# xmed-lab/GL-Fusion

Hardware: AMD Instinct MI355X
Metric: clips/sec fwd+bwd (B=4, 3 views x16x112x112) per GPU, weak scaling (higher is better)
Workload: dtype f32 (amax-scaled split-fp16 x3 MFMA, fp32 accumulate: fp32-equivalent); 1 GPU; C2: (B,V,T,H,W)=(4,3,16,112,112) per GPU, views 1/3/4, fp32 train() fwd + sum-BCE + bwd; global_batch_clips=4, frames_per_view_per_gpu=64, precision=f16x3, parallelism=single GPU, ranks_in_collective=1

## Files before the change

gl-fusion_amd/csrc/conv_api.hip:

```cpp
#include "gemm_common.h"
#include <cstring>

namespace {

int conv_out(int h, int k, int stride, int pad, int dil) { return (h + 2 * pad - dil * (k - 1) - 1) / stride + 1; }

unsigned tap_mask_of(int gather, int hd, int wd, int hs, int ws, int kh, int kw, int stride, int pad, int dil) {
    auto axis = [&](int nd, int ns, int k, bool* ok) {
        for (int t = 0; t < k; ++t) {
            ok[t] = false;
            for (int y = 0; y < nd && !ok[t]; ++y) {
                if (gather == 1) {
                    const int sy = y * stride - pad + t * dil;
                    ok[t] = sy >= 0 && sy < ns;
                } else {
                    const int v = y + pad - t * dil;
                    ok[t] = v >= 0 && v % stride == 0 && v / stride < ns;
                }
            }
        }
    };
    bool vy[32], vx[32];
    axis(hd, hs, kh, vy);
    axis(wd, ws, kw, vx);
// ... 30 lines not shown
        long long best = want;
        double best_score = -1.0;
        long long lo = want / 2 > 1 ? want / 2 : 1, up = want * 2;
        if (up > cap) up = cap;
        if (up > hi) up = hi;
        if (up < 1) up = 1;
        for (long long s = lo; s <= up; ++s) {
            const long long b = wg * s;
            const double score = (double)b / ((double)((b + 255) / 256) * 256.0) - 0.004 * (double)s;
            if (score > best_score) { best = s; best_score = score; }
        }
        want = best;
    }
    if (want > cap) want = cap;
    if (want > hi) want = hi;
    return (int)(want < 1 ? 1 : want);
}

int check_params(const glf_conv_params* p, const char* who) {
    GLF_REQUIRE(p != nullptr, GLF_ERR_NULL, "%s: null parameter block", who);
    GLF_REQUIRE(p->n > 0 && p->h > 0 && p->w > 0 && p->cin > 0 && p->cout > 0, GLF_ERR_BAD_SHAPE, "%s: extents must be > 0", who);
    GLF_REQUIRE(p->kh >= 1 && p->kw >= 1 && p->kh * p->kw <= 32 && p->stride >= 1 && p->dil >= 1 && p->pad >= 0, GLF_ERR_BAD_SHAPE,
                "%s: bad kernel geometry (kh*kw must be <= 32)", who);
    GLF_REQUIRE(p->precision >= 0 && p->precision <= 4, GLF_ERR_UNSUPPORTED, "%s: precision must be 0..4", who);
    GLF_REQUIRE(conv_out(p->h, p->kh, p->stride, p->pad, p->dil) > 0 && conv_out(p->w, p->kw, p->stride, p->pad, p->dil) > 0, GLF_ERR_BAD_SHAPE,
                "%s: empty output", who);
    return GLF_OK;
}

int effective_precision(const glf_conv_params* p) { return p->precision >= 1 ? p->precision - 1 : glf::precision(); }

constexpr double THR_FWD = 0.8, THR_DGRAD = 0.8, THR_DGRAD_F16 = 0.35, THR_WGRAD = 0.8, THR_REGION = 0.8;

void fill_geo(glf_gemm_params& g, const glf_conv_params* p, bool to_input, int ho, int wo) {
    g.n_img = p->n;
    g.kh = p->kh; g.kw = p->kw; g.stride = p->stride; g.pad = p->pad; g.dil = p->dil;
    if (to_input) { g.hs = ho; g.ws = wo; g.hd = p->h; g.wd = p->w; }
    else { g.hs = p->h; g.ws = p->w; g.hd = ho; g.wd = wo; }
}

}

extern "C" int glf_conv2d_plan(const glf_conv_params* p, int pass, glf_conv_plan* plan) {
    if (int rc = check_params(p, "conv2d_plan")) return rc;
    GLF_REQUIRE(plan != nullptr && pass >= 0 && pass <= 2, GLF_ERR_NULL, "conv2d_plan: plan missing or pass not in {0 fwd, 1 dgrad, 2 wgrad}");
    std::memset(plan, 0, sizeof(*plan));
    const int prec = effective_precision(p);
    const int ho = conv_out(p->h, p->kh, p->stride, p->pad, p->dil), wo = conv_out(p->w, p->kw, p->stride, p->pad, p->dil);
    const int taps = p->kh * p->kw;
    const bool plain = taps == 1 && p->stride == 1 && p->pad == 0;
    plan->ho = ho; plan->wo = wo; plan->taps = taps; plan->plain = plain; plan->split = 1;
    if (pass == 0 || pass == 2) {
        const unsigned mask = plain ? 1u : tap_mask_of(1, ho, wo, p->h, p->w, p->kh, p->kw, p->stride, p->pad, p->dil);
        const int kept = __builtin_popcount(mask);
        const double frac = (plain || p->stride != 1) ? 1.0 : rect_fraction(1, ho, wo, p->h, p->w, p->kw, p->pad, p->dil, mask);
        plan->tap_mask = mask; plan->kept_taps = kept;
        if (pass == 0) {
            plan->M = p->n * ho * wo; plan->N = p->cout; plan->K = p->cin;
            plan->rect = (!plain && taps > 1 && p->stride == 1 && kept > 1 && frac < THR_FWD) ? 1 : 0;
            plan->zero_fill = plan->rect == 1;
            plan->colstats_ok = prec >= 2 && p->cin % 32 == 0 && p->cout % 4 == 0 && plan->rect == 0;
        } else {
            const bool rect = !plain && taps > 1 && p->stride == 1 && kept > 1 && frac < THR_WGRAD;
            const long long rows_o = (long long)p->n * ho * wo;
            long long eff = rect ? (long long)((double)rows_o * frac) : rows_o;
            if (eff < 512) eff = 512;
            plan->M = p->cout; plan->N = p->cin; plan->K = (int)rows_o;
            plan->rect = rect ? 1 : 0;
            plan->split = tn_split(eff, p->cout, p->cin, kept, prec);
            if (rect) {
                long long s2 = (long long)((double)plan->split / (2.0 * (frac > 0.02 ? frac : 0.02)) + 0.999);
                if (s2 < plan->split) s2 = plan->split;
                const long long cap = rows_o / 512 > 1 ? rows_o / 512 : 1;
                if (s2 > cap) s2 = cap;
                if (s2 > 65535) s2 = 65535;
                plan->split = (int)(s2 < 1 ? 1 : s2);
            }
            plan->workspace_bytes = plan->split > 1 ? (int64_t)plan->split * kept * p->cout * p->cin * (int64_t)sizeof(float) : 0;
            plan->zero_fill = mask != ((taps == 32) ? 0xffffffffu : ((1u << taps) - 1u));
        }
    } else {
        const unsigned mask = plain ? 1u : tap_mask_of(2, p->h, p->w, ho, wo, p->kh, p->kw, p->stride, p->pad, p->dil);
        const int kept = __builtin_popcount(mask);
        const double frac = (plain || p->stride != 1) ? 1.0 : rect_fraction(2, p->h, p->w, ho, wo, p->kw, p->pad, p->dil, mask);
        plan->tap_mask = mask; plan->kept_taps = kept;
        plan->M = p->n * p->h * p->w; plan->N = p->cin; plan->K = p->cout;
        const bool region = prec >= 2 && !plain && kept > 1 && taps == 9 && p->kh == 3 && p->stride == 1 && p->pad == p->dil && ho == p->h &&
                            wo == p->w && p->cout % 32 == 0 && frac < THR_REGION;
        const double thr = prec >= 2 ? THR_DGRAD_F16 : THR_DGRAD;
        plan->rect = region ? 2 : ((!plain && taps > 1 && p->stride == 1 && kept > 1 && frac < thr) ? 1 : 0);
        plan->zero_fill = plan->rect == 1 || mask == 0;
    }
    return GLF_OK;
}

extern "C" int glf_conv2d_fwd(const float* x, const float* w_tap, const float* bias, float* y, const glf_conv_params* p, glf_stream_t s) {
    glf_conv_plan pl;
    if (int rc = glf_conv2d_plan(p, 0, &pl)) return rc;
    GLF_REQUIRE(x && w_tap && y, GLF_ERR_NULL, "conv2d_fwd: null argument");
    GLF_REQUIRE(!(pl.rect && bias), GLF_ERR_UNSUPPORTED, "conv2d_fwd: a bias on a conv that runs as per-tap rectangles is not built (none on the path)");
    GLF_REQUIRE(!p->colstats || pl.colstats_ok, GLF_ERR_UNSUPPORTED, "conv2d_fwd: colstats cannot be honoured for this conv / precision (see glf_conv_plan.colstats_ok)");
    if (pl.zero_fill) {
        hipError_t e = hipMemsetAsync(y, 0, (size_t)pl.M * pl.N * sizeof(float), glf::S(s));
        if (e != hipSuccess) return glf::fail(GLF_ERR_LAUNCH, "conv2d_fwd: hipMemsetAsync: %s", hipGetErrorString(e));
    }
    glf_gemm_params g;
    std::memset(&g, 0, sizeof(g));
    g.M = pl.M; g.N = pl.N; g.K = pl.K; g.lda = p->cin; g.ldb = p->cin; g.ldc = p->cout;
    g.taps = pl.taps; g.tap_mask = pl.tap_mask; g.tap_stride_b = (int64_t)p->cout * p->cin;
    g.gather = pl.plain ? 0 : 1;
    fill_geo(g, p, false, pl.ho, pl.wo);
    if (pl.plain) { g.n_img = 1; g.hs = g.ws = g.hd = g.wd = 1; g.kh = g.kw = 1; g.stride = 1; g.pad = 0; g.dil = 1; }
    g.batch = 1; g.alpha = 1.f; g.split = 1; g.rect = pl.rect;
    g.amax_a = p->amax_x; g.amax_b = p->amax_w; g.amax_c = p->amax_out; g.colstats = p->colstats; g.precision = p->precision;
    if (pl.rect == 1 && effective_precision(p) == 0) {
        for (unsigned mm = pl.tap_mask; mm; mm &= mm - 1) {
            g.tap_mask = mm & (~mm + 1u);
            if (int rc = glf_gemm_nt(x, w_tap, bias, y, &g, s)) return rc;
        }
        return GLF_OK;
    }
    return glf_gemm_nt(x, w_tap, bias, y, &g, s);
}

extern "C" int glf_conv2d_dgrad(const float* dy, const float* w_tap, const float* w_tap_t, float* dx, const glf_conv_params* p, glf_stream_t s) {
    glf_conv_plan pl;
    if (int rc = glf_conv2d_plan(p, 1, &pl)) return rc;
    GLF_REQUIRE(dy && dx && (w_tap || w_tap_t), GLF_ERR_NULL, "conv2d_dgrad: null argument");
    if (pl.zero_fill) {
        hipError_t e = hipMemsetAsync(dx, 0, (size_t)pl.M * pl.N * sizeof(float), glf::S(s));
        if (e != hipSuccess) return glf::fail(GLF_ERR_LAUNCH, "conv2d_dgrad: hipMemsetAsync: %s", hipGetErrorString(e));
        if (pl.tap_mask == 0) return GLF_OK;
    }
    const int prec = effective_precision(p);
    glf_gemm_params g;
    std::memset(&g, 0, sizeof(g));
    g.M = pl.M; g.N = pl.N; g.K = pl.K; g.lda = p->cout; g.ldc = p->cin;
    g.taps = pl.taps; g.tap_mask = pl.tap_mask; g.tap_stride_b = (int64_t)p->cout * p->cin;
    g.gather = pl.plain ? 0 : 2;
    fill_geo(g, p, true, pl.ho, pl.wo);
    if (pl.plain) { g.n_img = 1; g.hs = g.ws = g.hd = g.wd = 1; g.kh = g.kw = 1; g.stride = 1; g.pad = 0; g.dil = 1; }
    g.batch = 1; g.alpha = 1.f; g.split = 1; g.rect = pl.rect;
    g.amax_a = p->amax_dy; g.amax_b = p->amax_w; g.amax_c = p->amax_out; g.precision = p->precision;
    if (prec >= 1 && p->cout % 32 == 0 && w_tap_t) {
        g.ldb = p->cout;
        return glf_gemm_nt(dy, w_tap_t, nullptr, dx, &g, s);
// ... 35 lines not shown
```

gl-fusion_amd/csrc/gemm_common.h:

```cpp
#pragma once
#include "glf_common.h"

namespace glf {
struct Geo { int n_img, hs, ws, hd, wd, kh, kw, stride, pad, dil; };

struct GemmArgs {
    const float* A; const float* B; const float* bias; float* C;
    int M, N, K, lda, ldb, ldc, taps;
    unsigned tap_mask;
    long long tap_stride_b;
    int gather;
    Geo g;
    long long bsa, bsb, bsc;
    float alpha;
    int accumulate, split;
    int tiles_m, tiles_n;
    int vec_a, vec_b;
    int rect;
    const float* amax_a; const float* amax_b;
    const float* zeros;
    float* amax_c;
    double* colstats;
    float* colmax;
    float* partial;
// ... 69 lines not shown
}

__host__ __device__ inline void tap_rect(int gather, int tap, int kw, int pad, int dil, int hs, int ws, int hd, int wd,
                                         int& y0, int& y1, int& x0, int& x1) {
    const int ky = tap / kw, kx = tap - ky * kw;
    const int oy = (gather == 1) ? pad - ky * dil : ky * dil - pad;
    const int ox = (gather == 1) ? pad - kx * dil : kx * dil - pad;
    y0 = oy > 0 ? oy : 0;           y1 = hs + oy < hd ? hs + oy : hd;
    x0 = ox > 0 ? ox : 0;           x1 = ws + ox < wd ? ws + ox : wd;
    if (y1 < y0) y1 = y0;
    if (x1 < x0) x1 = x0;
}

__host__ __device__ inline void axis_band(int gather, int b, int d, int h, int& lo, int& hi, unsigned& taps) {
    int e1 = d < h - d ? d : h - d, e2 = d < h - d ? h - d : d;
    e1 = e1 < 0 ? 0 : (e1 > h ? h : e1);
    e2 = e2 < 0 ? 0 : (e2 > h ? h : e2);
    lo = b == 0 ? 0 : (b == 1 ? e1 : e2);
    hi = b == 0 ? e1 : (b == 1 ? e2 : h);
    const unsigned first = gather == 1 ? 0b110u : 0b011u, last = gather == 1 ? 0b011u : 0b110u;
    taps = b == 0 ? first : (b == 2 ? last : (d <= h - d ? 0b111u : 0b010u));
}
__host__ __device__ inline void region_of(int gather, int r, int d, int hd, int wd, int& y0, int& y1, int& x0, int& x1, unsigned& mask) {
    const int cell = (int)((0x8620'7531'4ull >> (4 * r)) & 0xf);
    unsigned ty, tx;
    axis_band(gather, cell / 3, d, hd, y0, y1, ty);
    axis_band(gather, cell % 3, d, wd, x0, x1, tx);
    mask = 0;
    for (int ky = 0; ky < 3; ++ky)
        for (int kx = 0; kx < 3; ++kx)
            if (((ty >> ky) & 1u) && ((tx >> kx) & 1u)) mask |= 1u << (ky * 3 + kx);
}

__device__ __forceinline__ float4 keep_if(bool c, const float4 v) {
    return make_float4(c ? v.x : 0.f, c ? v.y : 0.f, c ? v.z : 0.f, c ? v.w : 0.f);
}

__device__ __forceinline__ int xcd_remap(int bid, int nblk) {
    const int q = nblk >> 3, r = nblk & 7, xcd = bid & 7, idx = bid >> 3;
    return (xcd < r ? xcd * (q + 1) : r * (q + 1) + (xcd - r) * q) + idx;
}

int validate(const glf_gemm_params* p, const void* A, const void* B, const void* C) {
    GLF_REQUIRE(p && A && B && C, GLF_ERR_NULL, "gemm: null argument");
    GLF_REQUIRE(p->M > 0 && p->N > 0 && p->K > 0, GLF_ERR_BAD_SHAPE, "gemm: M,N,K must be > 0 (got %d,%d,%d)", p->M, p->N, p->K);
    GLF_REQUIRE(p->taps >= 1 && p->taps <= 32, GLF_ERR_BAD_SHAPE, "gemm: taps must be in [1,32] (got %d)", p->taps);
    GLF_REQUIRE(p->batch >= 1 && p->batch <= 65535, GLF_ERR_BAD_SHAPE, "gemm: batch out of range (%d)", p->batch);
    GLF_REQUIRE(p->gather >= 0 && p->gather <= 2, GLF_ERR_BAD_SHAPE, "gemm: gather must be 0,1,2");
    GLF_REQUIRE(p->precision >= 0 && p->precision <= 4, GLF_ERR_UNSUPPORTED, "gemm: precision must be 0 (process default), 1 (fp32), 2 (bf16x6), 3 (f16x3) or 4 (f16)");
    const unsigned full = p->taps == 32 ? 0xffffffffu : ((1u << p->taps) - 1u);
    GLF_REQUIRE((p->tap_mask & ~full) == 0, GLF_ERR_BAD_SHAPE, "gemm: tap_mask has bits beyond taps");
    if (p->gather) {
        GLF_REQUIRE(p->kh * p->kw == p->taps, GLF_ERR_BAD_SHAPE, "gemm: kh*kw != taps");
        GLF_REQUIRE(p->stride >= 1 && p->dil >= 1 && p->hs > 0 && p->ws > 0 && p->hd > 0 && p->wd > 0 && p->n_img > 0,
                    GLF_ERR_BAD_SHAPE, "gemm: bad conv geometry");
    } else {
        GLF_REQUIRE(p->taps == 1, GLF_ERR_BAD_SHAPE, "gemm: taps > 1 needs a gather mapping");
    }
    return GLF_OK;
}

GemmArgs make_args(const float* A, const float* B, const float* bias, float* C, const glf_gemm_params* p) {
    GemmArgs a;
    a.A = A; a.B = B; a.bias = bias; a.C = C;
    a.M = p->M; a.N = p->N; a.K = p->K; a.lda = p->lda; a.ldb = p->ldb; a.ldc = p->ldc; a.taps = p->taps;
    a.tap_mask = p->tap_mask; a.tap_stride_b = p->tap_stride_b; a.gather = p->gather;
// ... 37 lines not shown
```

gl-fusion_amd/csrc/gemm_f16s.hip:

```cpp
#include "gemm_common.h"
#include "split_f16.h"
#include <cstdlib>

namespace {

#define GLF_MFMA_F16(a, b, c) __builtin_amdgcn_mfma_f32_32x32x16_f16(a, b, c, 0, 0, 0)
#define GLF_ROW3(c0, c1, m0, m1, ah, al, b0h, b0l, b1h, b1l)  \
    c0 = GLF_MFMA_F16(ah, b0h, c0);                         \
    c1 = GLF_MFMA_F16(ah, b1h, c1);                         \
    if (NP == 3) {                                          \
        m0 = GLF_MFMA_F16(al, b0h, m0);                     \
        m1 = GLF_MFMA_F16(al, b1h, m1);                     \
        m0 = GLF_MFMA_F16(ah, b0l, m0);                     \
        m1 = GLF_MFMA_F16(ah, b1l, m1);                     \
    }

constexpr int BM8 = 256;
constexpr int NT8 = 512;
constexpr int WAVE_ROWS = 4;
#ifndef GLF_IL_ALL
#define GLF_IL_ALL 1
#endif
constexpr int PL_A8 = BM8 * 64, PL_B8 = BN * 64;
constexpr int BUF8 = 2 * PL_A8 + 2 * PL_B8;
// ... 20 lines not shown
    pow2_scale(args.amax_a, sc_a, inv_a);
    pow2_scale(args.amax_b, sc_b, inv_b);
    const float p_alpha = args.alpha * inv_a * inv_b;

    extern __shared__ __attribute__((aligned(16))) unsigned char smem_s[];
    unsigned* s_mask = reinterpret_cast<unsigned*>(smem_s + 3 * BUF8);
#if defined(GLF_STAMPS) && GLF_STAMPS == 2
    unsigned long long wg_t0 = __builtin_amdgcn_s_memtime(), wg_t1 = 0, wg_t2 = 0;
#endif

    const int tid = threadIdx.x, lane = tid & 63, wave = tid >> 6;
    const int wm = (wave >> 1) * 64, wn = (wave & 1) * 64;
    const int bid = xcd_remap(blockIdx.x, gridDim.x);
    int tn, tm;
    {
        const int gm = (args.flags >> 8) & 0xff;
        if (gm > 1) {
            const int tiles_m_all = gridDim.x / p_tiles_n;
            const int per_group = gm * p_tiles_n;
            const int grp = bid / per_group, in_grp = bid - grp * per_group;
            const int first_m = grp * gm;
            const int gsz = min(tiles_m_all - first_m, gm);
            tn = in_grp / gsz;
            tm = first_m + (in_grp - tn * gsz);
        } else {
            tn = bid % p_tiles_n;
            tm = bid / p_tiles_n;
        }
    }
    int pMe = pM;
    int r_y0 = 0, r_x0 = 0, r_h = g_hd, r_w = g_wd;
    unsigned mask = p_tap_mask;
    if (p_rect == 2) {
        bool found = false;
#pragma unroll
        for (int r = 0; r < 9; ++r) {
            int y0, y1, x0, x1;
            unsigned rm;
            region_of(p_gather, r, g_dil, g_hd, g_wd, y0, y1, x0, x1, rm);
            const int mt = g_nimg * (y1 - y0) * (x1 - x0);
            const int tiles = (mt + BM8 - 1) / BM8;
            if (!found) {
                if (tm < tiles) { found = true; mask = rm & p_tap_mask; pMe = mt; r_y0 = y0; r_x0 = x0; r_h = y1 - y0; r_w = x1 - x0; }
                else tm -= tiles;
            }
        }
        if (!found) return;
    } else if (p_rect) {
        for (unsigned mm = p_tap_mask; mm; mm &= mm - 1) {
            const int t = __ffs(mm) - 1;
            int y0, y1, x0, x1;
            tap_rect(p_gather, t, g_kw, g_pad, g_dil, g_hs, g_ws, g_hd, g_wd, y0, y1, x0, x1);
            const int mt = g_nimg * (y1 - y0) * (x1 - x0);
            const int tiles = (mt + BM8 - 1) / BM8;
            if (tm < tiles || (mm & (mm - 1)) == 0) { mask = 1u << t; pMe = mt; r_y0 = y0; r_x0 = x0; r_h = y1 - y0; r_w = x1 - x0; break; }
            tm -= tiles;
        }
    }
    const int bz = blockIdx.z;
    const float* __restrict__ A = p_A + (long long)bz * p_bsa;
    const float* __restrict__ B = p_B + (long long)bz * p_bsb;
    float* __restrict__ C = p_C + (long long)bz * p_bsc;

    const int ac = tid & 7, ar = tid >> 3;

    int a_n[4], a_y[4], a_x[4];
    long long a_off[4];
    {
        int cn = 0, cy = 0, cx = 0;
        if (GATHER) {
            const int m0 = tm * BM8 + ar, hw = r_h * r_w;
            cn = m0 / hw;
            const int rem = m0 - cn * hw;
            cy = rem / r_w; cx = rem - cy * r_w;
        }
#pragma unroll
        for (int j = 0; j < 4; ++j) {
            const int m = tm * BM8 + ar + 64 * j;
            if (GATHER) {
                if (m < pMe) { a_n[j] = cn; a_y[j] = r_y0 + cy; a_x[j] = r_x0 + cx; }
// ... 1253 lines not shown
    SET_ALL(false, 3) SET_ALL(true, 3) SET_ALL(false, 1) SET_ALL(true, 1)
#undef SET_ALL
#undef SET_TN
#undef SET_ROWS
#undef SET_ATTR
    return init_gemm_f16s4_attrs();
}

bool f16s_rows_ok(const GemmArgs& a) {
    return a.vec_a && a.vec_b && (a.K % BK) == 0 && a.K >= BK && a.K <= ZERO_PAGE_FLOATS && zero_page() != nullptr;
}
bool f16s_tn_ok(const GemmArgs& a) {
    return a.vec_a && a.vec_b && (a.M % 4) == 0 && (a.N % 4) == 0 && a.M >= 4 && a.N >= 4 &&
           a.M <= ZERO_PAGE_FLOATS && a.N <= ZERO_PAGE_FLOATS && zero_page() != nullptr;
}

#ifdef GLF_STAMPS
static void* stamps_buffer() {
    static void* p = [] { void* q = nullptr; (void)hipMalloc(&q, 8192); (void)hipMemset(q, 0, 8192); return q; }();
    return p;
}
extern "C" int glf_debug_stamps(void* host_out) {
    (void)hipDeviceSynchronize();
    return (int)hipMemcpy(host_out, stamps_buffer(), 8192, hipMemcpyDeviceToHost);
}
#endif

int launch_rows_f16s(const GemmArgs& a0, dim3 grid, bool gather, int nprod, hipStream_t s) {
    if (use_f16s4(a0)) return launch_rows_f16s4(a0, grid, gather, nprod, s);
    GemmArgs a = a0;
    a.zeros = zero_page();
    long long tiles_m = (a.M + BM8 - 1) / BM8;
    if (a.rect == 2) {
        tiles_m = 0;
        for (int r = 0; r < 9; ++r) {
            int y0, y1, x0, x1;
            unsigned rm;
            region_of(a.gather, r, a.g.dil, a.g.hd, a.g.wd, y0, y1, x0, x1, rm);
            tiles_m += ((long long)a.g.n_img * (y1 - y0) * (x1 - x0) + BM8 - 1) / BM8;
        }
    } else if (a.rect) {
        tiles_m = 0;
        for (unsigned mm = a.tap_mask; mm; mm &= mm - 1) {
            const int t = __builtin_ctz(mm);
            int y0, y1, x0, x1;
            tap_rect(a.gather, t, a.g.kw, a.g.pad, a.g.dil, a.g.hs, a.g.ws, a.g.hd, a.g.wd, y0, y1, x0, x1);
            tiles_m += ((long long)a.g.n_img * (y1 - y0) * (x1 - x0) + BM8 - 1) / BM8;
        }
    }
    a.tiles_m = (int)tiles_m;
    dim3 g2((unsigned)(tiles_m * a.tiles_n), 1, grid.z);
    const int group_m = (a.rect == 0 && a.tiles_n >= 8) ? 4 : 0;
    a.flags = (group_m & 0xff) << 8;
    const bool pa = a.a_presplit != 0, pb = a.b_presplit != 0;
#ifdef GLF_STAMPS
    a.partial = reinterpret_cast<float*>(stamps_buffer());
#endif
#define GLF_LAUNCH_ROWS(G, NP_, PA_, PB_) hipLaunchKernelGGL((gemm_rows_f16s8_kernel<G, NP_, false, PB_, PA_>), g2, dim3(NT8), SMEM_ROWS_H8, s, a)
#define GLF_ROWS_P(G, NP_)                                                                     \
    { if (pa && pb) GLF_LAUNCH_ROWS(G, NP_, true, true); else if (pa) GLF_LAUNCH_ROWS(G, NP_, true, false); \
      else if (pb) GLF_LAUNCH_ROWS(G, NP_, false, true); else GLF_LAUNCH_ROWS(G, NP_, false, false); }
    static const bool m16p = [] { const char* e = getenv("GLF_MFMA16_PRESPLIT"); return e ? e[0] != '0' : false; }();
    if (nprod == 3 && pa && pb && m16p) {
        if (gather) hipLaunchKernelGGL((gemm_rows_f16s8_kernel<true, 3, true, true, true>), g2, dim3(NT8), SMEM_ROWS_H8, s, a);
        else hipLaunchKernelGGL((gemm_rows_f16s8_kernel<false, 3, true, true, true>), g2, dim3(NT8), SMEM_ROWS_H8, s, a);
        return check_launch("gemm_nt(f16x3, 16x16x32, pre-split)");
    }
    if (nprod == 3) { if (gather) GLF_ROWS_P(true, 3) else GLF_ROWS_P(false, 3) }
    else { if (gather) GLF_ROWS_P(true, 1) else GLF_ROWS_P(false, 1) }
#undef GLF_ROWS_P
#undef GLF_LAUNCH_ROWS
    return check_launch("gemm_nt(f16x3, 256x128)");
}

int launch_tn_f16s(const GemmArgs& a0, dim3 grid, bool gather, int nprod, hipStream_t s) {
    GemmArgs a = a0;
    a.zeros = zero_page();
#ifdef GLF_STAMPS
    a.stamps = reinterpret_cast<unsigned long long*>(stamps_buffer());
#endif
    const bool pa = a.a_presplit != 0, pb = a.b_presplit != 0;
    static const bool small_on = [] { const char* e = getenv("GLF_TN_SMALL"); return e ? e[0] != '0' : true; }();
    const bool small = small_on && (a.M <= 64 || a.N <= 64) && a.M <= 256 && a.N <= 256;
    const bool wide = !small && a.M > BM;
// ... 33 lines not shown
```

gl-fusion_amd/csrc/gemm_f16s4.hip:

```cpp
#include "gemm_common.h"
#include "split_f16.h"
#include <cstdlib>

namespace {

#define GLF_MFMA_F16(a, b, c) __builtin_amdgcn_mfma_f32_32x32x16_f16(a, b, c, 0, 0, 0)
#define GLF_ROW3(c0, c1, m0, m1, ah, al, b0h, b0l, b1h, b1l)  \
    c0 = GLF_MFMA_F16(ah, b0h, c0);                         \
    c1 = GLF_MFMA_F16(ah, b1h, c1);                         \
    if (NP == 3) {                                          \
        m0 = GLF_MFMA_F16(al, b0h, m0);                     \
        m1 = GLF_MFMA_F16(al, b1h, m1);                     \
        m0 = GLF_MFMA_F16(ah, b0l, m0);                     \
        m1 = GLF_MFMA_F16(ah, b1l, m1);                     \
    }

constexpr int BM4 = 128;
constexpr int NT4 = 256;
constexpr int WAVE_ROWS = 2;
constexpr int RS4 = NT4 / 8;
constexpr int PL4 = 128 * 64;
constexpr int BUF4 = 4 * PL4;
constexpr size_t SMEM_ROWS_H4 = 2 * BUF4 + 16;

// ... 11 lines not shown
    const int g_stride = args.g.stride, g_pad = args.g.pad, g_dil = args.g.dil;
    const int g_nimg = args.g.n_img, p_rect = GATHER ? args.rect : 0;
    float sc_a, sc_b, inv_a, inv_b;
    pow2_scale(args.amax_a, sc_a, inv_a);
    pow2_scale(args.amax_b, sc_b, inv_b);
    const float p_alpha = args.alpha * inv_a * inv_b;

    extern __shared__ __attribute__((aligned(16))) unsigned char smem_s[];
    unsigned* s_mask = reinterpret_cast<unsigned*>(smem_s + 2 * BUF4);

    const int tid = threadIdx.x, lane = tid & 63, wave = tid >> 6;
    const int wm = (wave >> 1) * 64, wn = (wave & 1) * 64;
    const int bid = xcd_remap(blockIdx.x, gridDim.x);
    int tn, tm;
    {
        const int gm = (args.flags >> 8) & 0xff;
        if (gm > 1) {
            const int tiles_m_all = gridDim.x / p_tiles_n;
            const int per_group = gm * p_tiles_n;
            const int grp = bid / per_group, in_grp = bid - grp * per_group;
            const int first_m = grp * gm;
            const int gsz = min(tiles_m_all - first_m, gm);
            tn = in_grp / gsz;
            tm = first_m + (in_grp - tn * gsz);
        } else {
            tn = bid % p_tiles_n;
            tm = bid / p_tiles_n;
        }
    }
    int pMe = pM;
    int r_y0 = 0, r_x0 = 0, r_h = g_hd, r_w = g_wd;
    unsigned mask = p_tap_mask;
    if (p_rect == 2) {
        bool found = false;
#pragma unroll
        for (int r = 0; r < 9; ++r) {
            int y0, y1, x0, x1;
            unsigned rm;
            region_of(p_gather, r, g_dil, g_hd, g_wd, y0, y1, x0, x1, rm);
            const int mt = g_nimg * (y1 - y0) * (x1 - x0);
            const int tiles = (mt + BM4 - 1) / BM4;
            if (!found) {
                if (tm < tiles) { found = true; mask = rm & p_tap_mask; pMe = mt; r_y0 = y0; r_x0 = x0; r_h = y1 - y0; r_w = x1 - x0; }
                else tm -= tiles;
            }
        }
        if (!found) return;
    } else if (p_rect) {
        for (unsigned mm = p_tap_mask; mm; mm &= mm - 1) {
            const int t = __ffs(mm) - 1;
            int y0, y1, x0, x1;
            tap_rect(p_gather, t, g_kw, g_pad, g_dil, g_hs, g_ws, g_hd, g_wd, y0, y1, x0, x1);
            const int mt = g_nimg * (y1 - y0) * (x1 - x0);
            const int tiles = (mt + BM4 - 1) / BM4;
            if (tm < tiles || (mm & (mm - 1)) == 0) { mask = 1u << t; pMe = mt; r_y0 = y0; r_x0 = x0; r_h = y1 - y0; r_w = x1 - x0; break; }
            tm -= tiles;
        }
    }
    const int bz = blockIdx.z;
    const float* __restrict__ A = p_A + (long long)bz * p_bsa;
    const float* __restrict__ B = p_B + (long long)bz * p_bsb;
    float* __restrict__ C = p_C + (long long)bz * p_bsc;

    const int ac = tid & 7, ar = tid >> 3;

    int a_n[4], a_y[4], a_x[4];
    long long a_off[4];
    {
        int cn = 0, cy = 0, cx = 0;
        if (GATHER) {
            const int m0 = tm * BM4 + ar, hw = r_h * r_w;
            cn = m0 / hw;
            const int rem = m0 - cn * hw;
            cy = rem / r_w; cx = rem - cy * r_w;
        }
#pragma unroll
        for (int j = 0; j < 4; ++j) {
            const int m = tm * BM4 + ar + RS4 * j;
            if (GATHER) {
                if (m < pMe) { a_n[j] = cn; a_y[j] = r_y0 + cy; a_x[j] = r_x0 + cx; }
// ... 318 lines not shown
            }
        }
    }
    if (args.amax_c && p_rect != 1) {
#pragma unroll
        for (int o = 32; o > 0; o >>= 1) cmax = fmaxf(cmax, __shfl_xor(cmax, o, 64));
        if (lane == 0 && cmax > *reinterpret_cast<volatile float*>(args.amax_c))
            atomicMax(reinterpret_cast<unsigned*>(args.amax_c), __float_as_uint(cmax));
    }
}
}

namespace glf {

int init_gemm_f16s4_attrs() {
    hipError_t e;
#define SET_ATTR(fn)                                                                                     \
    e = hipFuncSetAttribute(reinterpret_cast<const void*>(fn), hipFuncAttributeMaxDynamicSharedMemorySize, (int)SMEM_ROWS_H4); \
    if (e != hipSuccess) return fail(GLF_ERR_LAUNCH, "hipFuncSetAttribute(" #fn "): %s", hipGetErrorString(e));
#define SET_P(G, NP_) SET_ATTR((gemm_rows_f16s4_kernel<G, NP_, false, false>)) SET_ATTR((gemm_rows_f16s4_kernel<G, NP_, true, false>)) \
                      SET_ATTR((gemm_rows_f16s4_kernel<G, NP_, false, true>)) SET_ATTR((gemm_rows_f16s4_kernel<G, NP_, true, true>))
    SET_P(false, 3) SET_P(true, 3) SET_P(false, 1) SET_P(true, 1)
#undef SET_P
#undef SET_ATTR
    return GLF_OK;
}

bool use_f16s4(const GemmArgs& a) {
    static const int mode = [] { const char* e = getenv("GLF_F16S4"); return e ? atoi(e) : 1; }();
    if (mode == 0) return false;
    if (mode == 2) return true;
    static const int kmax = [] { const char* e = getenv("GLF_F16S4_KMAX"); return e ? atoi(e) : 256; }();
    const long long kred = (long long)a.K * __builtin_popcount(a.tap_mask);
    return kred <= kmax;
}

int launch_rows_f16s4(const GemmArgs& a0, dim3 grid, bool gather, int nprod, hipStream_t s) {
    GemmArgs a = a0;
    a.zeros = zero_page();
    long long tiles_m = (a.M + BM4 - 1) / BM4;
    if (a.rect == 2) {
        tiles_m = 0;
        for (int r = 0; r < 9; ++r) {
            int y0, y1, x0, x1;
            unsigned rm;
            region_of(a.gather, r, a.g.dil, a.g.hd, a.g.wd, y0, y1, x0, x1, rm);
            tiles_m += ((long long)a.g.n_img * (y1 - y0) * (x1 - x0) + BM4 - 1) / BM4;
        }
    } else if (a.rect) {
        tiles_m = 0;
        for (unsigned mm = a.tap_mask; mm; mm &= mm - 1) {
            const int t = __builtin_ctz(mm);
            int y0, y1, x0, x1;
            tap_rect(a.gather, t, a.g.kw, a.g.pad, a.g.dil, a.g.hs, a.g.ws, a.g.hd, a.g.wd, y0, y1, x0, x1);
            tiles_m += ((long long)a.g.n_img * (y1 - y0) * (x1 - x0) + BM4 - 1) / BM4;
        }
    }
    a.tiles_m = (int)tiles_m;
    dim3 g2((unsigned)(tiles_m * a.tiles_n), 1, grid.z);
    a.flags = (a.rect == 0 && a.tiles_n >= 8 ? 4 : 0) << 8;
    const bool pa = a.a_presplit != 0, pb = a.b_presplit != 0;
#define GLF_L4(G, NP_, PA_, PB_) hipLaunchKernelGGL((gemm_rows_f16s4_kernel<G, NP_, PA_, PB_>), g2, dim3(NT4), SMEM_ROWS_H4, s, a)
#define GLF_L4P(G, NP_)                                                                   \
    { if (pa && pb) GLF_L4(G, NP_, true, true); else if (pa) GLF_L4(G, NP_, true, false); \
      else if (pb) GLF_L4(G, NP_, false, true); else GLF_L4(G, NP_, false, false); }
    if (nprod == 3) { if (gather) GLF_L4P(true, 3) else GLF_L4P(false, 3) }
    else { if (gather) GLF_L4P(true, 1) else GLF_L4P(false, 1) }
#undef GLF_L4P
#undef GLF_L4
    return check_launch("gemm_nt(f16x3, 128x128, 2 workgroups / CU)");
}

}
```

gl-fusion_amd/ops.py:

```python
from __future__ import annotations

import ctypes as C
import os
import weakref
from typing import List, Optional, Sequence, Tuple

import torch
from torch.autograd import Function
from torch.autograd.function import once_differentiable

from ._lib import GemmParams, WeightJob, WJ_AMAX, WJ_COPY, WJ_PACK, WJ_PASSES, WJ_PASS_OF, WJ_TAP_MAJOR, WJ_TAP_MAJOR_T, WJ_TRANSPOSE, WJ_ZERO, check, lib


def _p(t: Optional[torch.Tensor]):
    return None if t is None else C.c_void_p(t.data_ptr())


def _stream():
    return C.c_void_p(torch.cuda.current_stream().cuda_stream)


def _chk(t: torch.Tensor, name: str = "tensor") -> torch.Tensor:
    if not isinstance(t, torch.Tensor) or not t.is_cuda or t.dtype != torch.float32:
        raise RuntimeError(
# ... 668 lines not shown


_rect_cache = {}


def rect_fraction(gather: int, hd: int, wd: int, hs: int, ws: int, kh: int, kw: int, pad: int, dil: int, mask: int) -> float:
    key = (gather, hd, wd, hs, ws, kh, kw, pad, dil, mask)
    f = _rect_cache.get(key)
    if f is None:
        tot, n = 0, 0
        for t in range(kh * kw):
            if not (mask >> t) & 1:
                continue
            ky, kx = divmod(t, kw)
            oy = pad - ky * dil if gather == 1 else ky * dil - pad
            ox = pad - kx * dil if gather == 1 else kx * dil - pad
            rh = max(0, min(hs + oy, hd) - max(oy, 0))
            rw = max(0, min(ws + ox, wd) - max(ox, 0))
            tot += rh * rw
            n += 1
        f = tot / max(1, n * hd * wd)
        _rect_cache[key] = f
    return f


RECT_THRESHOLD = {"fwd": 0.8, "dgrad": 0.8, "wgrad": 0.8, "dgrad_f16x3": 0.35, "region": 0.8}


def region_mode(taps: int, kh: int, stride: int, pad: int, dil: int, h: int, w: int, ho: int, wo: int, k: int, frac: float) -> bool:
    return (os.environ.get("GLF_REGION", "1") != "0" and _PREC[0] >= 2 and taps == 9 and kh == 3 and stride == 1 and pad == dil and h == ho and w == wo
            and k % 32 == 0 and frac < RECT_THRESHOLD["region"])


def _rect_thr(which: str) -> float:
    if which == "dgrad" and _PREC[0] >= 2:
        return RECT_THRESHOLD["dgrad_f16x3"]
    return RECT_THRESHOLD[which]


def _conv_out(h: int, k: int, stride: int, pad: int, dil: int) -> int:
    return (h + 2 * pad - dil * (k - 1) - 1) // stride + 1


class Conv2dFn(Function):

    @staticmethod
    def forward(ctx, x, weight, bias, stride: int, pad: int, dil: int, colstats=None):
        _chk(x, "conv input"); _chk(weight, "conv weight")
        x = _contig(x)
        n, h, w, cin = x.shape
        cout, cin_w, kh, kw = weight.shape
        if cin_w != cin:
            raise RuntimeError(f"conv2d: input has {cin} channels, weight expects {cin_w}")
        ho, wo = _conv_out(h, kh, stride, pad, dil), _conv_out(w, kw, stride, pad, dil)
        if ho <= 0 or wo <= 0:
            raise RuntimeError("conv2d: empty output")
        taps = kh * kw
        wt = tap_major(weight)
        y = torch.empty(n, ho, wo, cout, dtype=torch.float32, device=x.device)
        plain = taps == 1 and stride == 1 and pad == 0
        geo = (n, h, w, ho, wo, kh, kw, stride, pad, dil)
        mask = 1 if plain else tap_mask(1, ho, wo, h, w, kh, kw, stride, pad, dil)
        rect = (not plain and taps > 1 and stride == 1 and bias is None and bin(mask).count("1") > 1
                and rect_fraction(1, ho, wo, h, w, kh, kw, pad, dil, mask) < _rect_thr("fwd"))
        if rect:
            zero_(y)
            if colstats is not None:
                raise RuntimeError("conv2d: fused column statistics are not available for a conv evaluated as per-tap rectangles")
        am_w, am_x = amax_of(weight), amax_of(x)
        x_pk = packed_only(x)
        skinny = plain and n * ho * wo <= 64 and cout >= 64 and cin % 16 == 0 and not x_pk and colstats is None
        ok = nt_presplit_ok(cin, cin, cin) and not skinny
        if x_pk and not (ok and am_x is not None and takes_packed_input(weight)):
            raise RuntimeError("glfusion_amd: a packed-only activation reached a convolution that cannot consume it")
        ok_x = ok and (cout * bin(mask).count("1") >= PRESPLIT_MIN_COLS or packed_hit(x, am_x) is not None)
        xa, pa = (x, True) if x_pk else pick(x, act_packed(x, am_x) if ok_x else None, ok_x)
        wb, pb = pick(wt, weight_packed(wt, weight, "w", am_w) if ok else None, ok)
        masks = [1 << t_ for t_ in range(taps) if (mask >> t_) & 1] if (rect and _PREC[0] == 0) else [mask]
        for mk in masks:
            gemm("nt", xa, wb, y, M=n * ho * wo, N=cout, K=cin, lda=cin, ldb=cin, ldc=cout, bias=bias,
                 taps=taps, mask=mk, tap_stride_b=cout * cin, gather=0 if plain else 1, geo=None if plain else geo, rect=rect,
                 amax_a=am_x, amax_b=am_w, colstats=colstats, colmax=getattr(colstats, "_glf_colmax", None), a_packed=pa, b_packed=pb)
        ctx.save_for_backward(x, wt)
        ctx.x_packed = (xa, am_x) if (pa and (x_pk or packed_hit(x, am_x) is not None)) else None
        ctx.join = getattr(x, "_glf_join", None) if plain else None
        ctx.weight_ref = weight
        ctx.cfg = (n, h, w, cin, cout, kh, kw, ho, wo, stride, pad, dil, plain, bias is not None, tuple(weight.shape))
        return y

    @staticmethod
    @once_differentiable
    def backward(ctx, dy):
        x, wt = ctx.saved_tensors
        n, h, w, cin, cout, kh, kw, ho, wo, stride, pad, dil, plain, has_bias, wshape = ctx.cfg
        dy = _contig(dy)
        taps = kh * kw
        rows_o = n * ho * wo
        dx = dw = db = None
        am_dy, am_w = amax_of(dy), amax_of(ctx.weight_ref)
        dy_pk = packed_only(dy)
        if dy_pk and (has_bias or am_dy is None or not (split_mode() and cout % 32 == 0)):
            raise RuntimeError("glfusion_amd: a packed-only gradient reached a convolution that cannot consume it")
        def dgrad():
            dx = None
            if True:
                mask = 1 if plain else tap_mask(2, h, w, ho, wo, kh, kw, stride, pad, dil)
                if mask == 0:
                    dx = zeros(x.shape, device=x.device)
                else:
                    frac = 1.0 if plain or stride != 1 else rect_fraction(2, h, w, ho, wo, kh, kw, pad, dil, mask)
                    if not plain and bin(mask).count("1") > 1 and region_mode(taps, kh, stride, pad, dil, ho, wo, h, w, cout, frac):
# ... 78 lines not shown
                dw.record_stream(cur)
        else:
            if ctx.needs_input_grad[0]:
                dx = dgrad()
            if ctx.needs_input_grad[1]:
                dw = wgrad()
        if has_bias and ctx.needs_input_grad[2]:
            db = colsum(dy, rows_o, cout)
        return dx, dw, db, None, None, None, None


def conv2d(x, weight, bias=None, stride: int = 1, pad: int = 0, dil: int = 1, colstats=None):
    if _is16(x):
        from . import ops16
        return ops16.conv2d(x, weight, bias, stride, pad, dil, colstats)
    return Conv2dFn.apply(x, weight, bias, stride, pad, dil, colstats)


def conv_stats_fusable(weight, stride: int, pad: int, dil: int, h: int, w: int, dtype=None) -> bool:
    if _S16[0]:
        return dtype == torch.bfloat16 and weight.shape[1] % 64 == 0 and weight.shape[0] % 64 == 0
    if _PREC[0] < 2:
        return False
    cout, cin, kh, kw = weight.shape
    if cin % 32 != 0 or cout % 4 != 0:
        return False
    taps = kh * kw
    if taps == 1 and stride == 1 and pad == 0:
        return True
    ho, wo = _conv_out(h, kh, stride, pad, dil), _conv_out(w, kw, stride, pad, dil)
    if ho <= 0 or wo <= 0:
        return False
    mask = tap_mask(1, ho, wo, h, w, kh, kw, stride, pad, dil)
    rect = (taps > 1 and stride == 1 and bin(mask).count("1") > 1
            and rect_fraction(1, ho, wo, h, w, kh, kw, pad, dil, mask) < _rect_thr("fwd"))
    return not rect


class ConvCatFn(Function):

    @staticmethod
    def forward(ctx, weight, bias, *xs):
        _chk(weight, "weight")
        cout, ctot = weight.shape[0], weight.shape[1]
        w2 = _contig(weight.detach()).view(cout, ctot)
        rows = xs[0].numel() // xs[0].shape[-1]
        t0 = _chk(xs[0], "input")
        offs = [0]
        for t in xs:
            offs.append(offs[-1] + t.shape[-1])
        ctx.cat = (offs[-1] == ctot and not t0.is_contiguous() and t0.stride(-1) == 1 and t0.stride(-2) == ctot
                   and all(_chk(t, "input").stride() == t0.stride() and t.shape[:-1] == t0.shape[:-1]
                           and t.data_ptr() == t0.data_ptr() + 4 * o for t, o in zip(xs, offs)))
        if ctx.cat:
            y = torch.empty(*t0.shape[:-1], cout, dtype=torch.float32, device=t0.device)
            am_w = amax_of(weight)
            ok = nt_presplit_ok(ctot, ctot, ctot)
            wb, pb = pick(w2, weight_packed(w2, weight, "w", am_w) if ok else None, ok)
            gemm("nt", t0, wb, y, M=rows, N=cout, K=ctot, lda=ctot, ldb=ctot, ldc=cout, bias=bias,
                 amax_a=amax_of(t0), amax_b=am_w, b_packed=pb)
            ctx.save_for_backward(w2, *xs)
            ctx.wshape = tuple(weight.shape)
            ctx.weight_ref = weight
            ctx.has_bias = bias is not None
            return y
        xs = [_contig(_chk(t, "input")) for t in xs]
        y = torch.empty(*xs[0].shape[:-1], cout, dtype=torch.float32, device=xs[0].device)
        off = 0
        for i, t in enumerate(xs):
# ... 1032 lines not shown
```

Baseline: 16.55 clips/s.

## Run forward rect convs as nine-region tiles ordered by tap count

```diff
diff --git a/gl-fusion_amd/csrc/conv_api.hip b/gl-fusion_amd/csrc/conv_api.hip
--- a/gl-fusion_amd/csrc/conv_api.hip
+++ b/gl-fusion_amd/csrc/conv_api.hip
@@ -86,6 +86,10 @@
 
 constexpr double THR_FWD = 0.8, THR_DGRAD = 0.8, THR_DGRAD_F16 = 0.35, THR_WGRAD = 0.8, THR_REGION = 0.8;
 
+bool fwd_regions(const glf_conv_params* p, int prec, int ho, int wo) {
+    return prec >= 2 && p->cout >= 128 && p->kh == 3 && p->kw == 3 && p->stride == 1 && p->pad == p->dil && ho == p->h && wo == p->w && p->cin % 32 == 0;
+}
+
 void fill_geo(glf_gemm_params& g, const glf_conv_params* p, bool to_input, int ho, int wo) {
     g.n_img = p->n;
     g.kh = p->kh; g.kw = p->kw; g.stride = p->stride; g.pad = p->pad; g.dil = p->dil;
@@ -112,8 +116,9 @@
         if (pass == 0) {
             plan->M = p->n * ho * wo; plan->N = p->cout; plan->K = p->cin;
             plan->rect = (!plain && taps > 1 && p->stride == 1 && kept > 1 && frac < THR_FWD) ? 1 : 0;
-            plan->zero_fill = plan->rect == 1;
-            plan->colstats_ok = prec >= 2 && p->cin % 32 == 0 && p->cout % 4 == 0 && plan->rect == 0;
+            const bool regions = plan->rect == 1 && fwd_regions(p, prec, ho, wo);
+            plan->zero_fill = plan->rect == 1 && !regions;
+            plan->colstats_ok = prec >= 2 && p->cin % 32 == 0 && p->cout % 4 == 0 && (plan->rect == 0 || regions);
         } else {
             const bool rect = !plain && taps > 1 && p->stride == 1 && kept > 1 && frac < THR_WGRAD;
             const long long rows_o = (long long)p->n * ho * wo;
@@ -165,7 +170,8 @@
     g.gather = pl.plain ? 0 : 1;
     fill_geo(g, p, false, pl.ho, pl.wo);
     if (pl.plain) { g.n_img = 1; g.hs = g.ws = g.hd = g.wd = 1; g.kh = g.kw = 1; g.stride = 1; g.pad = 0; g.dil = 1; }
-    g.batch = 1; g.alpha = 1.f; g.split = 1; g.rect = pl.rect;
+    g.batch = 1; g.alpha = 1.f; g.split = 1;
+    g.rect = (pl.rect == 1 && !pl.zero_fill) ? 2 : pl.rect;
     g.amax_a = p->amax_x; g.amax_b = p->amax_w; g.amax_c = p->amax_out; g.colstats = p->colstats; g.precision = p->precision;
     if (pl.rect == 1 && effective_precision(p) == 0) {
         for (unsigned mm = pl.tap_mask; mm; mm &= mm - 1) {
diff --git a/gl-fusion_amd/csrc/gemm_common.h b/gl-fusion_amd/csrc/gemm_common.h
--- a/gl-fusion_amd/csrc/gemm_common.h
+++ b/gl-fusion_amd/csrc/gemm_common.h
@@ -125,6 +125,46 @@
             if (((ty >> ky) & 1u) && ((tx >> kx) & 1u)) mask |= 1u << (ky * 3 + kx);
 }
 
+__host__ __device__ inline bool region_tile(int gather, int d, int hd, int wd, int n_img, unsigned tap_mask, int bm, int tiles_n, int b,
+                                            int& region, int& tm, int& tn) {
+    const int idx = b >> 3, k = idx / tiles_n;
+    tn = idx - k * tiles_n;
+    int t = k * 8 + (b & 7);
+    int len[9], til[9];
+#pragma unroll
+    for (int r = 0; r < 9; ++r) {
+        int y0, y1, x0, x1;
+        unsigned rm;
+        region_of(gather, r, d, hd, wd, y0, y1, x0, x1, rm);
+        len[r] = __builtin_popcount(rm & tap_mask);
+        til[r] = (n_img * (y1 - y0) * (x1 - x0) + bm - 1) / bm;
+    }
+    region = -1;
+#pragma unroll
+    for (int i = 0; i < 7; ++i) {
+        const int L = (int)((0x0123469u >> (4 * i)) & 0xf);
+#pragma unroll
+        for (int r = 0; r < 9; ++r)
+            if (region < 0 && len[r] == L) {
+                if (t < til[r]) region = r;
+                else t -= til[r];
+            }
+    }
+    tm = t;
+    return region >= 0;
+}
+inline long long region_tiles_m(int gather, int d, int hd, int wd, int n_img, int bm) {
+    long long tiles = 0;
+    for (int r = 0; r < 9; ++r) {
+        int y0, y1, x0, x1;
+        unsigned rm;
+        region_of(gather, r, d, hd, wd, y0, y1, x0, x1, rm);
+        tiles += ((long long)n_img * (y1 - y0) * (x1 - x0) + bm - 1) / bm;
+    }
+    return tiles;
+}
+inline long long region_grid_blocks(long long tiles_m, int tiles_n) { return 8 * ((tiles_m + 7) / 8) * tiles_n; }
+
 __device__ __forceinline__ float4 keep_if(bool c, const float4 v) {
     return make_float4(c ? v.x : 0.f, c ? v.y : 0.f, c ? v.z : 0.f, c ? v.w : 0.f);
 }
diff --git a/gl-fusion_amd/csrc/gemm_f16s.hip b/gl-fusion_amd/csrc/gemm_f16s.hip
--- a/gl-fusion_amd/csrc/gemm_f16s.hip
+++ b/gl-fusion_amd/csrc/gemm_f16s.hip
@@ -76,20 +76,12 @@
     int r_y0 = 0, r_x0 = 0, r_h = g_hd, r_w = g_wd;
     unsigned mask = p_tap_mask;
     if (p_rect == 2) {
-        bool found = false;
-#pragma unroll
-        for (int r = 0; r < 9; ++r) {
-            int y0, y1, x0, x1;
-            unsigned rm;
-            region_of(p_gather, r, g_dil, g_hd, g_wd, y0, y1, x0, x1, rm);
-            const int mt = g_nimg * (y1 - y0) * (x1 - x0);
-            const int tiles = (mt + BM8 - 1) / BM8;
-            if (!found) {
-                if (tm < tiles) { found = true; mask = rm & p_tap_mask; pMe = mt; r_y0 = y0; r_x0 = x0; r_h = y1 - y0; r_w = x1 - x0; }
-                else tm -= tiles;
-            }
-        }
-        if (!found) return;
+        int r;
+        if (!region_tile(p_gather, g_dil, g_hd, g_wd, g_nimg, p_tap_mask, BM8, p_tiles_n, (int)blockIdx.x, r, tm, tn)) return;
+        int y0, y1, x0, x1;
+        unsigned rm;
+        region_of(p_gather, r, g_dil, g_hd, g_wd, y0, y1, x0, x1, rm);
+        mask = rm & p_tap_mask; pMe = g_nimg * (y1 - y0) * (x1 - x0); r_y0 = y0; r_x0 = x0; r_h = y1 - y0; r_w = x1 - x0;
     } else if (p_rect) {
         for (unsigned mm = p_tap_mask; mm; mm &= mm - 1) {
             const int t = __ffs(mm) - 1;
@@ -1409,13 +1401,7 @@
     a.zeros = zero_page();
     long long tiles_m = (a.M + BM8 - 1) / BM8;
     if (a.rect == 2) {
-        tiles_m = 0;
-        for (int r = 0; r < 9; ++r) {
-            int y0, y1, x0, x1;
-            unsigned rm;
-            region_of(a.gather, r, a.g.dil, a.g.hd, a.g.wd, y0, y1, x0, x1, rm);
-            tiles_m += ((long long)a.g.n_img * (y1 - y0) * (x1 - x0) + BM8 - 1) / BM8;
-        }
+        tiles_m = region_tiles_m(a.gather, a.g.dil, a.g.hd, a.g.wd, a.g.n_img, BM8);
     } else if (a.rect) {
         tiles_m = 0;
         for (unsigned mm = a.tap_mask; mm; mm &= mm - 1) {
@@ -1426,7 +1412,7 @@
         }
     }
     a.tiles_m = (int)tiles_m;
-    dim3 g2((unsigned)(tiles_m * a.tiles_n), 1, grid.z);
+    dim3 g2((unsigned)(a.rect == 2 ? region_grid_blocks(tiles_m, a.tiles_n) : tiles_m * a.tiles_n), 1, grid.z);
     const int group_m = (a.rect == 0 && a.tiles_n >= 8) ? 4 : 0;
     a.flags = (group_m & 0xff) << 8;
     const bool pa = a.a_presplit != 0, pb = a.b_presplit != 0;
diff --git a/gl-fusion_amd/csrc/gemm_f16s4.hip b/gl-fusion_amd/csrc/gemm_f16s4.hip
--- a/gl-fusion_amd/csrc/gemm_f16s4.hip
+++ b/gl-fusion_amd/csrc/gemm_f16s4.hip
@@ -67,20 +67,12 @@
     int r_y0 = 0, r_x0 = 0, r_h = g_hd, r_w = g_wd;
     unsigned mask = p_tap_mask;
     if (p_rect == 2) {
-        bool found = false;
-#pragma unroll
-        for (int r = 0; r < 9; ++r) {
-            int y0, y1, x0, x1;
-            unsigned rm;
-            region_of(p_gather, r, g_dil, g_hd, g_wd, y0, y1, x0, x1, rm);
-            const int mt = g_nimg * (y1 - y0) * (x1 - x0);
-            const int tiles = (mt + BM4 - 1) / BM4;
-            if (!found) {
-                if (tm < tiles) { found = true; mask = rm & p_tap_mask; pMe = mt; r_y0 = y0; r_x0 = x0; r_h = y1 - y0; r_w = x1 - x0; }
-                else tm -= tiles;
-            }
-        }
-        if (!found) return;
+        int r;
+        if (!region_tile(p_gather, g_dil, g_hd, g_wd, g_nimg, p_tap_mask, BM4, p_tiles_n, (int)blockIdx.x, r, tm, tn)) return;
+        int y0, y1, x0, x1;
+        unsigned rm;
+        region_of(p_gather, r, g_dil, g_hd, g_wd, y0, y1, x0, x1, rm);
+        mask = rm & p_tap_mask; pMe = g_nimg * (y1 - y0) * (x1 - x0); r_y0 = y0; r_x0 = x0; r_h = y1 - y0; r_w = x1 - x0;
     } else if (p_rect) {
         for (unsigned mm = p_tap_mask; mm; mm &= mm - 1) {
             const int t = __ffs(mm) - 1;
@@ -465,7 +457,12 @@
     if (mode == 2) return true;
     static const int kmax = [] { const char* e = getenv("GLF_F16S4_KMAX"); return e ? atoi(e) : 256; }();
     const long long kred = (long long)a.K * __builtin_popcount(a.tap_mask);
-    return kred <= kmax;
+    if (kred <= kmax) return true;
+    if (a.rect == 2 && a.gather != 0) {
+        const long long t8 = region_tiles_m(a.gather, a.g.dil, a.g.hd, a.g.wd, a.g.n_img, 256) * a.tiles_n;
+        return t8 < 2 * 256;
+    }
+    return false;
 }
 
 int launch_rows_f16s4(const GemmArgs& a0, dim3 grid, bool gather, int nprod, hipStream_t s) {
@@ -473,13 +470,7 @@
     a.zeros = zero_page();
     long long tiles_m = (a.M + BM4 - 1) / BM4;
     if (a.rect == 2) {
-        tiles_m = 0;
-        for (int r = 0; r < 9; ++r) {
-            int y0, y1, x0, x1;
-            unsigned rm;
-            region_of(a.gather, r, a.g.dil, a.g.hd, a.g.wd, y0, y1, x0, x1, rm);
-            tiles_m += ((long long)a.g.n_img * (y1 - y0) * (x1 - x0) + BM4 - 1) / BM4;
-        }
+        tiles_m = region_tiles_m(a.gather, a.g.dil, a.g.hd, a.g.wd, a.g.n_img, BM4);
     } else if (a.rect) {
         tiles_m = 0;
         for (unsigned mm = a.tap_mask; mm; mm &= mm - 1) {
@@ -490,7 +481,7 @@
         }
     }
     a.tiles_m = (int)tiles_m;
-    dim3 g2((unsigned)(tiles_m * a.tiles_n), 1, grid.z);
+    dim3 g2((unsigned)(a.rect == 2 ? region_grid_blocks(tiles_m, a.tiles_n) : tiles_m * a.tiles_n), 1, grid.z);
     a.flags = (a.rect == 0 && a.tiles_n >= 8 ? 4 : 0) << 8;
     const bool pa = a.a_presplit != 0, pb = a.b_presplit != 0;
 #define GLF_L4(G, NP_, PA_, PB_) hipLaunchKernelGGL((gemm_rows_f16s4_kernel<G, NP_, PA_, PB_>), g2, dim3(NT4), SMEM_ROWS_H4, s, a)
diff --git a/gl-fusion_amd/ops.py b/gl-fusion_amd/ops.py
--- a/gl-fusion_amd/ops.py
+++ b/gl-fusion_amd/ops.py
@@ -724,6 +724,10 @@
             and k % 32 == 0 and frac < RECT_THRESHOLD["region"])
 
 
+def fwd_region_mode(taps: int, kh: int, stride: int, pad: int, dil: int, h: int, w: int, ho: int, wo: int, cin: int, cout: int, frac: float) -> bool:
+    return cout >= 128 and region_mode(taps, kh, stride, pad, dil, h, w, ho, wo, cin, frac)
+
+
 def _rect_thr(which: str) -> float:
     if which == "dgrad" and _PREC[0] >= 2:
         return RECT_THRESHOLD["dgrad_f16x3"]
@@ -755,7 +759,9 @@
         mask = 1 if plain else tap_mask(1, ho, wo, h, w, kh, kw, stride, pad, dil)
         rect = (not plain and taps > 1 and stride == 1 and bias is None and bin(mask).count("1") > 1
                 and rect_fraction(1, ho, wo, h, w, kh, kw, pad, dil, mask) < _rect_thr("fwd"))
-        if rect:
+        if rect and fwd_region_mode(taps, kh, stride, pad, dil, h, w, ho, wo, cin, cout, rect_fraction(1, ho, wo, h, w, kh, kw, pad, dil, mask)):
+            rect = 2
+        elif rect:
             zero_(y)
             if colstats is not None:
                 raise RuntimeError("conv2d: fused column statistics are not available for a conv evaluated as per-tap rectangles")
@@ -768,7 +774,7 @@
         ok_x = ok and (cout * bin(mask).count("1") >= PRESPLIT_MIN_COLS or packed_hit(x, am_x) is not None)
         xa, pa = (x, True) if x_pk else pick(x, act_packed(x, am_x) if ok_x else None, ok_x)
         wb, pb = pick(wt, weight_packed(wt, weight, "w", am_w) if ok else None, ok)
-        masks = [1 << t_ for t_ in range(taps) if (mask >> t_) & 1] if (rect and _PREC[0] == 0) else [mask]
+        masks = [1 << t_ for t_ in range(taps) if (mask >> t_) & 1] if (rect == 1 and _PREC[0] == 0) else [mask]
         for mk in masks:
             gemm("nt", xa, wb, y, M=n * ho * wo, N=cout, K=cin, lda=cin, ldb=cin, ldc=cout, bias=bias,
                  taps=taps, mask=mk, tap_stride_b=cout * cin, gather=0 if plain else 1, geo=None if plain else geo, rect=rect,
@@ -913,9 +919,9 @@
     if ho <= 0 or wo <= 0:
         return False
     mask = tap_mask(1, ho, wo, h, w, kh, kw, stride, pad, dil)
-    rect = (taps > 1 and stride == 1 and bin(mask).count("1") > 1
-            and rect_fraction(1, ho, wo, h, w, kh, kw, pad, dil, mask) < _rect_thr("fwd"))
-    return not rect
+    frac = rect_fraction(1, ho, wo, h, w, kh, kw, pad, dil, mask)
+    rect = taps > 1 and stride == 1 and bin(mask).count("1") > 1 and frac < _rect_thr("fwd")
+    return not rect or fwd_region_mode(taps, kh, stride, pad, dil, h, w, ho, wo, cin, cout, frac)
 
 
 class ConvCatFn(Function):
```

Result: no change. 16.61 clips/s, median of 6 (+0.3%).
